# haliphinx/TCE-RVOS

Hardware: AMD Instinct MI355X
Metric: clips/s (T=5, 360×640, Swin-T) at 1/2/4/8 MI355X; mask IoU vs ref (higher is better)
Workload: dtype f32 (3xf16-split MFMA, f32 accumulate); 1 GPU; swin_t_p4w7 T=5 360x640 + 32-token text, B=1 clip per forward, flags --with_box_refine --binary --f_token 8 --qtrans (BASELINE config 2); clips_in_flight_per_gpu=1, clips_per_forward=1, same_clip_in_group=False, ranks_per_gpu=1, parallelism=clip-sharded x1

## Files before the change

include/tce_rvos.h:

```cpp
#ifndef TCE_RVOS_H
#define TCE_RVOS_H
#include <stdint.h>

#ifdef __cplusplus
extern "C" {
#endif

typedef void* tceStream;

int tce_abi_version(void);
const char* tce_last_error(void);

typedef struct {
  const float* A;
  const float* A2;
  const float* W;
  const float* bias;
  const float* res;
  float* C;
  int32_t M, N, K;
  int32_t lda, lda2, ldw, ldc, ldres;
  int32_t act, res_mode;
  int32_t batch;
  int64_t sA, sA2, sW, sBias, sC, sRes;
// ... 114 lines not shown
int tce_embed_ln_f32(const int64_t* ids, const int64_t* pos_ids, const float* word, const float* pos, const float* type0,
                     const float* gamma, const float* beta, float* out, int32_t L, int32_t C, float eps, int32_t pad_id,
                     tceStream stream);
int tce_embed_ln_seqs_f32(const int64_t* ids, const float* word, const float* pos, const float* type0, const float* gamma,
                          const float* beta, float* out, int32_t nseq, int32_t seq_len, int32_t C, float eps, int32_t pad_id,
                          tceStream stream);
int tce_mha_small64_f32(const float* qkv, float* out, int32_t L, int32_t nheads, float scale, tceStream stream);
int tce_tanh_f32(const float* x, float* out, int64_t n, tceStream stream);

int32_t tce_thin_linear_splits(int32_t M, int32_t N, int32_t K);
int tce_thin_partials_f32(const float* x, int64_t ldx, int32_t xsplits, const float* bias_x, int32_t act_x, const float* W,
                          int64_t ldw, float* ws, int32_t M, int32_t N, int32_t K, tceStream stream);
int tce_splitk_reduce_f32(const float* ws, int32_t splits, int32_t M, int32_t N, const float* bias, int32_t act, const float* res,
                          int32_t ldres, int32_t res_mode, float* C, int32_t ldc, const float* gamma, const float* beta, float eps,
                          tceStream stream);
int tce_mha_small64_splits_f32(const float* qkv_planes, int32_t splits, const float* bias, float* out, int32_t L, int32_t nheads,
                               float scale, tceStream stream);
int tce_mha_small64_seqs_f32(const float* qkv_planes, int32_t splits, const float* bias, float* out, int32_t nseq, int32_t L,
                             int32_t nheads, float scale, tceStream stream);
int tce_mha_small64_lens_f32(const float* qkv_planes, int32_t splits, const float* bias, float* out, int32_t nseq, int32_t L,
                             int32_t nheads, float scale, const int32_t* lens, tceStream stream);
int tce_caption_lens_f32(const int64_t* ids, int32_t nseq, int32_t Lmax, int32_t pad_id, int32_t D, int32_t* lens, uint8_t* kmask,
                         float* pos, tceStream stream);

int64_t tce_ffn_packed_bytes(int32_t C, int32_t Hd);
int tce_ffn_pack_f32(const float* W1, const float* b1, const float* W2, void* packed, int32_t C, int32_t Hd,
                     tceStream stream);
int tce_ffn_pack_batched_f32(const float* W1, const float* b1, const float* W2, void* packed, int32_t C, int32_t Hd,
                             int32_t batch, tceStream stream);
int tce_ffn_fused_f32(const float* x, int64_t ldx, const void* packed, const float* b2, const float* g_in,
                      const float* be_in, float eps_in, const float* g_out, const float* be_out, float eps_out,
                      float* out, int64_t ldo, int32_t M, int32_t C, int32_t Hd, int32_t act, tceStream stream);
int64_t tce_ffn_split_ws_floats(int32_t M, int32_t C, int32_t Hd, int32_t act);
int32_t tce_ffn_split_counters(int32_t M, int32_t C, int32_t Hd, int32_t act);
int tce_ffn_fused_split_f32(const float* x, int64_t ldx, const void* packed, const float* b2, const float* g_in, const float* be_in,
                            float eps_in, const float* g_out, const float* be_out, float eps_out, float* out, int64_t ldo, int32_t M,
                            int32_t C, int32_t Hd, int32_t act, float* ws, int64_t ws_floats, int32_t* counters, int32_t n_counters,
                            tceStream stream);

typedef struct {
  const float* x;
  const float* a2;
  const void* packed;
  const float* bias;
  const float* res;
  float* out;
  const float *g_in, *be_in, *g_out, *be_out;
  int64_t ldx, lda2, ldres, ldo;
  int64_t sX, sA2, sRes, sOut;
  int32_t M, N, K, batch, a2_rows, act, res_mode;
  float eps_in, eps_out;
} tceRowLinArgs;
int64_t tce_rowlin_packed_bytes(int32_t N, int32_t K);
int tce_rowlin_pack_f32(const float* W, int64_t ldw, void* packed, int32_t N, int32_t K, tceStream stream);
int tce_rowlin_f32(const tceRowLinArgs* args, tceStream stream);

int64_t tce_conv3x3_packed_bytes(int32_t Cin, int32_t N);
int tce_conv3x3_pack_f32(const float* w, void* packed, int32_t Cin, int32_t N, tceStream stream);
int tce_conv3x3_f32(const float* x, int64_t ldx, const void* packed, const float* bias, float* out, int64_t ldo, int32_t T,
                    int32_t H, int32_t W, int32_t Cin, int32_t N, tceStream stream);
int64_t tce_conv3x3_split_ws_floats(int32_t M, int32_t Cin, int32_t N);
int32_t tce_conv3x3_split_pieces(int32_t M, int32_t Cin, int32_t N);
int32_t tce_conv3x3_split_kstep(int32_t pieces, int32_t s);
int tce_conv3x3_split_f32(const float* x, int64_t ldx, const void* packed, const float* bias, float* out, int64_t ldo, int32_t T,
                          int32_t H, int32_t W, int32_t Cin, int32_t N, float* ws, int64_t ws_floats, tceStream stream);

// ... 77 lines not shown
```

tce-rvos_amd/_lib.py:

```python
import ctypes as C
import os

HERE = os.path.dirname(os.path.abspath(__file__))
LIB_PATH = os.environ.get("TCE_LIB") or os.path.join(HERE, "lib", "libtce_rvos.so")

c_f = C.c_void_p
i32, i64, f32 = C.c_int32, C.c_int64, C.c_float


class GemmArgs(C.Structure):
    _fields_ = [("A", c_f), ("A2", c_f), ("W", c_f), ("bias", c_f), ("res", c_f), ("C", c_f),
                ("M", i32), ("N", i32), ("K", i32),
                ("lda", i32), ("lda2", i32), ("ldw", i32), ("ldc", i32), ("ldres", i32),
                ("act", i32), ("res_mode", i32), ("batch", i32),
                ("sA", i64), ("sA2", i64), ("sW", i64), ("sBias", i64), ("sC", i64), ("sRes", i64),
                ("conv", i32), ("T", i32), ("H", i32), ("Wd", i32), ("Cin", i32), ("Ho", i32), ("Wo", i32),
                ("kh", i32), ("kw", i32), ("stride", i32), ("pad", i32)]


class RowLinArgs(C.Structure):
    _fields_ = [("x", c_f), ("a2", c_f), ("packed", c_f), ("bias", c_f), ("res", c_f), ("out", c_f),
                ("g_in", c_f), ("be_in", c_f), ("g_out", c_f), ("be_out", c_f),
                ("ldx", i64), ("lda2", i64), ("ldres", i64), ("ldo", i64),
                ("sX", i64), ("sA2", i64), ("sRes", i64), ("sOut", i64),
# ... 64 lines not shown
    "tce_ms_deform_attn_forward_f32": (i32, [c_f, c_f, c_f, c_f, c_f, c_f, i32, i32, i32, i32, i32, i32, i32, c_f]),
    "tce_ms_deform_attn_backward_f32": (i32, [c_f, c_f, c_f, c_f, c_f, c_f, c_f, c_f, c_f, i32, i32, i32, i32, i32, i32, i32, c_f]),
    "tce_msda_fused_f32": (i32, [c_f, c_f, c_f, c_f, C.POINTER(i32), i32, i32, i32, i32, i32, i32, i32, i32, c_f]),
    "tce_msda_fused_valid_f32": (i32, [c_f, c_f, c_f, c_f, C.POINTER(i32), C.POINTER(i32), i32, i32, i32, i32, i32, i32, i32,
                                       i32, c_f]),
    "tce_msda_fewq_raw_f32": (i32, [c_f, c_f, c_f, c_f, c_f, c_f, C.POINTER(i32), C.POINTER(i32), i32, i32, i32, i32, i32, i32, i32,
                                    i32, c_f]),
    "tce_contrastive_f32": (i32, [c_f, c_f, c_f, c_f, i32, i32, i32, i32, c_f]),
    "tce_pos_sine2d_f32": (i32, [c_f, c_f, i32, i32, i32, i32, c_f]),
    "tce_pos_sine2d_valid_f32": (i32, [c_f, c_f, i32, i32, i32, i32, i32, i32, c_f]),
    "tce_resize_nearest_f32": (i32, [c_f, c_f, c_f, i32, i32, i32, i32, i32, i32, c_f]),
    "tce_resize_bilinear_f32": (i32, [c_f, c_f, c_f, i32, i32, i32, i32, i32, i32, c_f]),
    "tce_resize_bilinear_ln_f32": (i32, [c_f, c_f, c_f, c_f, f32, c_f, i32, i32, i32, i32, i32, i32, c_f]),
    "tce_add_f32": (i32, [c_f, c_f, c_f, i64, i64, c_f]),
    "tce_tile_f32": (i32, [c_f, c_f, i64, i64, c_f]),
    "tce_sigmoid_f32": (i32, [c_f, c_f, i64, c_f]),
    "tce_copy_segments": (i32, [C.POINTER(CopySeg), i32, c_f]),
    "tce_box_refine_f32": (i32, [c_f, c_f, c_f, i32, i32, c_f]),
    "tce_mask_pack_f32": (i32, [c_f, c_f, c_f, i32, i32, i32, i32, c_f]),
    "tce_mask_tail_f32": (i32, [c_f, c_f, c_f, i32, c_f, i32, i32, i32, i32, i32, f32, f32, i32, c_f]),
    "tce_select_masks_u8": (i32, [c_f, c_f, c_f, c_f, i32, i32, i32, i32, i32, i32, i32, f32, c_f]),
    "tce_embed_ln_f32": (i32, [c_f, c_f, c_f, c_f, c_f, c_f, c_f, c_f, i32, i32, f32, i32, c_f]),
    "tce_mha_small64_f32": (i32, [c_f, c_f, i32, i32, f32, c_f]),
    "tce_mha_small64_seqs_f32": (i32, [c_f, i32, c_f, c_f, i32, i32, i32, f32, c_f]),
    "tce_embed_ln_seqs_f32": (i32, [c_f, c_f, c_f, c_f, c_f, c_f, c_f, i32, i32, i32, f32, i32, c_f]),
    "tce_mha_small64_lens_f32": (i32, [c_f, i32, c_f, c_f, i32, i32, i32, f32, c_f, c_f]),
    "tce_caption_lens_f32": (i32, [c_f, i32, i32, i32, i32, c_f, c_f, c_f, c_f]),
    "tce_tanh_f32": (i32, [c_f, c_f, i64, c_f]),
    "tce_ffn_packed_bytes": (i64, [i32, i32]),
    "tce_ffn_pack_f32": (i32, [c_f, c_f, c_f, c_f, i32, i32, c_f]),
    "tce_ffn_fused_f32": (i32, [c_f, i64, c_f, c_f, c_f, c_f, f32, c_f, c_f, f32, c_f, i64, i32, i32, i32, i32, c_f]),
    "tce_ffn_split_ws_floats": (i64, [i32, i32, i32, i32]),
    "tce_ffn_split_counters": (i32, [i32, i32, i32, i32]),
    "tce_ffn_fused_split_f32": (i32, [c_f, i64, c_f, c_f, c_f, c_f, f32, c_f, c_f, f32, c_f, i64, i32, i32, i32, i32, c_f, i64, c_f, i32, c_f]),
    "tce_xattn_prepare_f32": (i32, [c_f, c_f, c_f, c_f, c_f, c_f, c_f, i32, i32, i32, c_f]),
    "tce_ffn_pack_batched_f32": (i32, [c_f, c_f, c_f, c_f, i32, i32, i32, c_f]),
    "tce_xattn_fused_f32": (i32, [C.POINTER(XattnArgs), c_f]),
    "tce_xattn_ffn_fused_f32": (i32, [C.POINTER(XattnArgs), C.POINTER(XattnFfnArgs), c_f]),
    "tce_ffn_pack_chain_f32": (i32, [c_f, c_f, c_f, c_f, i32, i32, c_f]),
    "tce_xattn_pack_f32": (i32, [c_f, c_f, c_f, c_f, c_f, i32, i32, i32, c_f]),
    "tce_xattn_prepare_lens_f32": (i32, [c_f, c_f, c_f, c_f, c_f, c_f, c_f, i32, i32, i32, c_f, c_f]),
    "tce_xattn_pack_lens_f32": (i32, [c_f, c_f, c_f, c_f, c_f, i32, i32, i32, c_f, c_f]),
    "tce_rowlin_packed_bytes": (i64, [i32, i32]),
    "tce_rowlin_pack_f32": (i32, [c_f, i64, c_f, i32, i32, c_f]),
    "tce_rowlin_f32": (i32, [C.POINTER(RowLinArgs), c_f]),
    "tce_conv3x3_packed_bytes": (i64, [i32, i32]),
    "tce_conv3x3_pack_f32": (i32, [c_f, c_f, i32, i32, c_f]),
    "tce_conv3x3_f32": (i32, [c_f, i64, c_f, c_f, c_f, i64, i32, i32, i32, i32, i32, c_f]),
    "tce_conv3x3_split_ws_floats": (i64, [i32, i32, i32]),
    "tce_conv3x3_split_pieces": (i32, [i32, i32, i32]),
    "tce_conv3x3_split_kstep": (i32, [i32, i32]),
    "tce_conv3x3_split_f32": (i32, [c_f, i64, c_f, c_f, c_f, i64, i32, i32, i32, i32, i32, c_f, i64, c_f]),
    "tce_fewrow_linear_f32": (i32, [C.POINTER(FewRowArgs), c_f]),
    "tce_thin_linear_splits": (i32, [i32, i32, i32]),
    "tce_thin_partials_f32": (i32, [c_f, i64, i32, c_f, i32, c_f, i64, c_f, i32, i32, i32, c_f]),
    "tce_splitk_reduce_f32": (i32, [c_f, i32, i32, i32, c_f, i32, c_f, i32, i32, c_f, i32, c_f, c_f, f32, c_f]),
    "tce_mha_small64_splits_f32": (i32, [c_f, i32, c_f, c_f, i32, i32, f32, c_f]),
    "tce_swin_attn_packed_bytes": (i64, [i32]),
    "tce_swin_attn_pack_f32": (i32, [c_f, c_f, c_f, i32, c_f]),
    "tce_swin_attn_fused_f32": (i32, [c_f, i64, c_f, c_f, c_f, c_f, c_f, c_f, f32, c_f, i64, i32, i32, i32, i32, i32, c_f]),
    "tce_graph_begin": (i32, [c_f]),
    "tce_graph_end": (i32, [c_f, C.POINTER(C.c_void_p)]),
    "tce_graph_launch": (i32, [C.c_void_p, c_f]),
    "tce_graph_destroy": (i32, [C.c_void_p]),
    "tce_graph_group": (i32, [C.POINTER(C.c_void_p), i32, C.POINTER(C.c_void_p)]),
}
# ... 56 lines not shown
```

tce-rvos_amd/csrc/chain.hip:

```cpp
#include "common.h"
#include "gemm_epilogue.h"
#include "frag.h"
#include "../../include/tce_rvos.h"
#include "../../include/tce_rvos_debug.h"

namespace {

#ifndef FFN_ABL
#define FFN_ABL 0
#endif
static __device__ long long* g_ffn_stamps = nullptr;


template <int K, bool HAS_A2 = true>
__device__ __forceinline__ void load_x_frags(const float* __restrict__ x, const long long ldx,
                                             const float* __restrict__ a2, const long long lda2, const int a2_rows,
                                             const int m0, const int M, float* __restrict__ wt, const int lane,
                                             const float* __restrict__ g_in, const float* __restrict__ be_in,
                                             const float eps, h16x8 (&xh)[K / 16], h16x8 (&xl)[K / 16],
                                             const int single = 0) {
  constexpr int NP = K / 32;
  const int cr = lane >> 3, cp = (lane & 7) * 4;
  const int r = lane & 31, hf = lane >> 5;
  f32x4 v[NP][4];
// ... 199 lines not shown
      const f32x4 gv = *reinterpret_cast<const f32x4*>(gamma + 32 * t + 8 * g + 4 * hf);
      const f32x4 bv = *reinterpret_cast<const f32x4*>(beta + 32 * t + 8 * g + 4 * hf);
#pragma unroll
      for (int c = 0; c < 4; ++c) acc[t][4 * g + c] = (acc[t][4 * g + c] - mean) * rstd * gv[c] + bv[c];
    }
}

struct FfnArgs {
  const float* x;
  const unsigned char* wpk;
  const float* b2;
  const float *g_in, *be_in, *g_out, *be_out;
  float* out;
  long long ldx, ldo;
  const float *a2, *res;
  long long lda2, ldres, sX, sRes, sOut, sW;
  int a2_rows, res_mode;
  int M, NI;
  float eps_in, eps_out;
  int* range_flag;
  int single;
  int wdiv;
  const unsigned char* wpk2;
  const float *b22, *g_out2, *be_out2;
  float* mid;
  long long ldmid, sMid;
  int NI2;
  float eps_out2;
  float* ws;
  int* cnt;
  int sp_p, sp_k0, sp_k1, nblk;
};

template <int C, int WAVES, int ACT, bool SINGLE, int ACT2 = 0, bool SPLIT = false>
__global__ void __launch_bounds__(64 * WAVES, (WAVES == 4 && C <= 128) ? 2 : WAVES / 4) ffn_fused_kernel(const FfnArgs p) {
  static_assert(!(SPLIT && ACT2 != 0), "a chain is not split");
  constexpr int KS = C / 16, NT = C / 32;
  constexpr bool HALF = WAVES == 4 && C <= 128;
  constexpr int PWAVES = HALF ? 8 : WAVES;
  constexpr int P = (1 + 2 * KS + 4 * NT + PWAVES - 1) / PWAVES * PWAVES;
  constexpr int SLOTS = P / WAVES;
  static_assert(!(HALF && (SPLIT || ACT2 != 0)), "the half form is the plain kernel");
  constexpr int STAGE = P * PIECE;
  constexpr int STEPS = KS + 2 * NT;
  static_assert(SLOTS <= STEPS, "more DMA slots than loop steps");
  static_assert(2 * STAGE + (HALF ? 0 : WAVES * WT_BYTES) <= (HALF ? 80 : 160) * 1024, "ring + staging tiles do not fit the LDS");
  static_assert(!HALF || WAVES * WT_BYTES <= STAGE, "the half form's staging tiles alias one ring stage");
  __shared__ __attribute__((aligned(16))) unsigned char smem[2 * STAGE + (HALF ? 0 : WAVES * WT_BYTES) + (SPLIT ? 16 : 0)];

  const int tid = threadIdx.x, lane = tid & 63;
  const int wave = __builtin_amdgcn_readfirstlane(tid >> 6);
  const int hf = lane >> 5;

  if (p.NI < 0) reinterpret_cast<u32x4*>(smem)[tid] = u32x4{0u, 0u, 0u, 0u};

  long long* const stamps = (g_ffn_stamps && blockIdx.x < 1024 && blockIdx.y == 0 && tid == 0) ? g_ffn_stamps + blockIdx.x * 8 : nullptr;
  if (stamps) {
    stamps[0] = (long long)__builtin_amdgcn_s_memtime();
    stamps[4] = (long long)__builtin_amdgcn_s_memrealtime();
  }
  const unsigned char* wp = p.wpk + (long long)(blockIdx.y / p.wdiv) * p.sW + (long long)wave * PIECE;
  const unsigned char* const wp0 = wp;
  const unsigned voff = lane * 16;
  const unsigned wbase = wave * PIECE;
  auto dma = [&](int stage, int q) {
    const unsigned char* src = wp;
    if constexpr (ACT2 != 0 || SPLIT) {
      const unsigned long long u = (unsigned long long)wp;
      const unsigned lo = __builtin_amdgcn_readfirstlane((unsigned)u), hi = __builtin_amdgcn_readfirstlane((unsigned)(u >> 32));
      src = (const unsigned char*)(((unsigned long long)hi << 32) | lo);
      glds16(src, voff, (unsigned)__builtin_amdgcn_readfirstlane((int)(wbase + (unsigned)(stage * STAGE + q * WAVES * PIECE))));
      wp += WAVES * PIECE;
      return;
    }
    glds16(src, voff, wbase + (unsigned)(stage * STAGE + q * WAVES * PIECE));
    wp += WAVES * PIECE;
  };
  const float* const xb = p.x + blockIdx.y * p.sX;
  const float* const resb = p.res ? p.res + blockIdx.y * p.sRes : xb;
  const long long ldres = p.res ? p.ldres : p.ldx;
  float* const outb = p.out + blockIdx.y * p.sOut;
  float* const wt = reinterpret_cast<float*>(smem + (HALF ? STAGE : 2 * STAGE) + wave * WT_BYTES);
  tce_amax_t amax = 0;
  constexpr int single = SINGLE;
  constexpr int NPC = SPLIT ? 2 : 1;
  for (int pc = 0; pc < NPC; ++pc) {
  int blk = blockIdx.x, nit = p.NI;
  if constexpr (SPLIT) {
    const int q = p.sp_p + 1, g = blockIdx.x / q, i = blockIdx.x - g * q;
    int c0 = 0;
    if (pc == 0) {
      if (i == p.sp_p) continue;
      blk = g * p.sp_p + i;
      nit = (i == 0 ? p.sp_k0 : p.sp_k1) + 1;
    } else {
      if (i == 0) continue;
      blk = g * p.sp_p + i - 1;
      c0 = i == 1 ? p.sp_k0 : p.sp_k1;
      nit = p.NI - c0;
    }
    if (blk >= p.nblk) continue;
    wp = wp0 + (long long)c0 * (P * PIECE);
  }
#pragma unroll
  for (int q = 0; q < SLOTS; ++q) dma(0, q);

  const int m0 = blk * (32 * WAVES) + wave * 32;
  h16x8 xh[KS], xl[KS];
  load_x_frags<C, (ACT >= 3)>(xb, p.ldx, p.a2, p.lda2, p.a2_rows, m0, p.M, wt, lane, p.g_in, p.be_in, p.eps_in, xh, xl, SINGLE);

  f32x16 oacc[NT];
#pragma unroll
  for (int t = 0; t < NT; ++t)
#pragma unroll
    for (int i = 0; i < 16; ++i) oacc[t][i] = 0.f;
  h16x8 hh0, hl0, hh1, hl1;
#pragma unroll
  for (int j = 0; j < 8; ++j) hh0[j] = hl0[j] = hh1[j] = hl1[j] = (_Float16)0.f;

  asm volatile("s_waitcnt vmcnt(0)" ::: "memory");
// ... 552 lines not shown
inline FfnSplitPlan ffn_split_plan(int M, int C, int Hd, int batch) {
  FfnSplitPlan best;
  const int B = tce_cdiv(M, 32 * ffn_waves(C)), NC = Hd / 32, CUS = tce_cu_count();
  if (C != 256 || NC < 24 || batch < 1) return best;
  const int OVP = 3, OVF = 4;
  auto rounds = [&](long long wgs) { return (double)((wgs + CUS - 1) / CUS); };
  double best_cost = 0.75 * rounds((long long)B * batch) * (NC + 1 + OVP + OVF);
  for (int p = 1; p <= 2; ++p) {
    const int wd = p == 1 ? 0 : (p * NC - 2 * (1 + OVP)) / (p + 1), ws_ = p == 1 ? (NC + 1) / 2 : wd + 1 + OVP;
    int k[2] = {ws_, 0};
    bool ok = ws_ >= 1 && ws_ <= NC - 1;
    for (int i = 1; i < p && ok; ++i) {
      k[i] = wd - (NC - k[i - 1]);
      ok = k[i] >= 1 && k[i] <= NC - 1;
    }
    if (!ok) continue;
    const int busiest = ws_ > NC - k[p - 1] ? ws_ : NC - k[p - 1];
    const double cost = rounds((long long)tce_cdiv(B, p) * (p + 1) * batch) * (busiest + 1 + OVP + OVF);
    if (cost < best_cost) {
      best_cost = cost;
      best.p = p;
      for (int i = 0; i < 2; ++i) best.k[i] = k[i];
    }
  }
  if (best.p) {
    best.nblk = B;
    best.ws_floats = (long long)batch * B * 2 * (32 * ffn_waves(C)) * C;
  }
  return best;
}

static int g_ffn_half = 0;

template <int C, int WAVES>
void ffn_launch(const FfnArgs& a, int act, hipStream_t s, int batch = 1) {
  if constexpr (C == 256) {
    if (a.sp_p > 0 && act == 1) {
      const dim3 grid(tce_cdiv(a.nblk, a.sp_p) * (a.sp_p + 1), batch), block(64 * WAVES);
      if (a.single) hipLaunchKernelGGL((ffn_fused_kernel<C, WAVES, 1, true, 0, true>), grid, block, 0, s, a);
      else hipLaunchKernelGGL((ffn_fused_kernel<C, WAVES, 1, false, 0, true>), grid, block, 0, s, a);
      return;
    }
  }
  if constexpr (C <= 128 && WAVES == 8) {
    const long long b8 = (long long)tce_cdiv(a.M, 256) * batch, b4 = (long long)tce_cdiv(a.M, 128) * batch, cus = tce_cu_count();
    const double c8 = (double)((b8 + cus - 1) / cus);
    const long long rem = b4 % (2 * cus);
    const double c4 = (double)(b4 / (2 * cus)) + (rem == 0 ? 0.0 : rem <= cus ? 0.5 : 1.0);
    if (act == 2 && g_ffn_half >= 0 && (g_ffn_half > 0 || c4 <= c8)) {
      const dim3 grid(tce_cdiv(a.M, 128), batch), block(256);
      if (a.single) hipLaunchKernelGGL((ffn_fused_kernel<C, 4, 2, true>), grid, block, 0, s, a);
      else hipLaunchKernelGGL((ffn_fused_kernel<C, 4, 2, false>), grid, block, 0, s, a);
      return;
    }
  }
  const dim3 grid(tce_cdiv(a.M, 32 * WAVES), batch), block(64 * WAVES);
  if (a.single) {
    if (act == 1) hipLaunchKernelGGL((ffn_fused_kernel<C, WAVES, 1, true>), grid, block, 0, s, a);
    else if (act == 2) hipLaunchKernelGGL((ffn_fused_kernel<C, WAVES, 2, true>), grid, block, 0, s, a);
  } else {
    if (act == 1) hipLaunchKernelGGL((ffn_fused_kernel<C, WAVES, 1, false>), grid, block, 0, s, a);
    else if (act == 2) hipLaunchKernelGGL((ffn_fused_kernel<C, WAVES, 2, false>), grid, block, 0, s, a);
  }
}

__global__ void __launch_bounds__(256) xattn_prepare_kernel(const float* __restrict__ k, const float* __restrict__ v,
                                                            const float* __restrict__ wqT, const float* __restrict__ wo,
                                                            float* __restrict__ W1, float* __restrict__ b1,
                                                            float* __restrict__ W2, const int L, const int G,
                                                            const int* __restrict__ lens) {
  constexpr int C = 256, HD = 32;
  const int Hd = 8 * G;
  const int Lb = lens ? min(lens[blockIdx.y], L) : L;
  k += (long long)blockIdx.y * L * C;
  v += (long long)blockIdx.y * L * C;
  W1 += (long long)blockIdx.y * Hd * C;
  b1 += (long long)blockIdx.y * Hd;
  W2 += (long long)blockIdx.y * C * Hd;
  const int idx = blockIdx.x * 256 + threadIdx.x;
  if (idx < Hd * C) {
    const int r = idx / C, i = idx - r * C, h = r / G, j = r - h * G;
    float a = 0.f;
    if (j < Lb) {
      const f32x4* kp = reinterpret_cast<const f32x4*>(k + j * C + h * HD);
      const f32x4* wp = reinterpret_cast<const f32x4*>(wqT + (long long)i * C + h * HD);
// ... 513 lines not shown
  hipLaunchKernelGGL(ffn_pack_kernel, dim3(tce_cdiv(units, 256)), dim3(256), 0, (hipStream_t)stream, W1, b1, W2,
                     (unsigned char*)packed, C, Hd, ffn_pieces(C), units, tce_gemm_single_pass(), 1);
  TCE_CHECK_LAUNCH("tce_ffn_pack_chain_f32");
  return TCE_OK;
}

extern "C" int tce_ffn_fused_f32(const float* x, int64_t ldx, const void* packed, const float* b2, const float* g_in,
                                 const float* be_in, float eps_in, const float* g_out, const float* be_out,
                                 float eps_out, float* out, int64_t ldo, int32_t M, int32_t C, int32_t Hd, int32_t act,
                                 tceStream stream) {
  TCE_CHECK_ARG(ffn_shape_ok(C, Hd), "tce_ffn_fused_f32: unsupported shape C=%d hidden=%d", C, Hd);
  TCE_CHECK_ARG(M > 0 && x && packed && b2 && out, "tce_ffn_fused_f32: null pointer or M <= 0");
  TCE_CHECK_ARG(act == 1 || act == 2, "tce_ffn_fused_f32: act must be 1 (ReLU) or 2 (GELU)");
  TCE_CHECK_ARG(ldx >= C && ldo >= C && ldx % 4 == 0 && ldo % 4 == 0, "tce_ffn_fused_f32: bad row pitch");
  TCE_CHECK_ARG(tce_aligned16(x) && tce_aligned16(out) && tce_aligned16(packed) && tce_aligned16(b2),
                "tce_ffn_fused_f32: x/out/packed/b2 must be 16-byte aligned");
  TCE_CHECK_ARG((!g_in || (be_in && tce_aligned16(g_in) && tce_aligned16(be_in))) &&
                    (!g_out || (be_out && tce_aligned16(g_out) && tce_aligned16(be_out))),
                "tce_ffn_fused_f32: LayerNorm gamma/beta must come in pairs, 16-byte aligned");
  FfnArgs a = {};
  a.x = x; a.wpk = (const unsigned char*)packed; a.b2 = b2; a.res_mode = 1;
  a.g_in = g_in; a.be_in = be_in; a.g_out = g_out; a.be_out = be_out;
  a.out = out; a.ldx = ldx; a.ldo = ldo; a.M = M; a.NI = Hd / 32 + 1; a.eps_in = eps_in; a.eps_out = eps_out; a.range_flag = tce_range_flag(); a.single = tce_gemm_single_pass();
  a.wdiv = 1;
  hipStream_t s = (hipStream_t)stream;
  if (C == 256) ffn_launch<256, 4>(a, act, s);
  else if (C == 192) ffn_launch<192, 4>(a, act, s);
  else if (C == 128) ffn_launch<128, 8>(a, act, s);
  else ffn_launch<96, 8>(a, act, s);
  TCE_CHECK_LAUNCH("tce_ffn_fused_f32");
  return TCE_OK;
}

extern "C" int tce_debug_ffn_set_half(int32_t mode) {
  TCE_CHECK_ARG(mode >= -1 && mode <= 1, "tce_debug_ffn_set_half: -1 (never), 0 (automatic) or 1 (always)");
  g_ffn_half = mode;
  return TCE_OK;
}

extern "C" int64_t tce_ffn_split_ws_floats(int32_t M, int32_t C, int32_t Hd, int32_t act) {
  if (M <= 0 || !ffn_shape_ok(C, Hd) || act != 1) return 0;
  return ffn_split_plan(M, C, Hd, 1).ws_floats;
}

extern "C" int32_t tce_ffn_split_counters(int32_t M, int32_t C, int32_t Hd, int32_t act) {
  if (M <= 0 || !ffn_shape_ok(C, Hd) || act != 1) return 0;
  return ffn_split_plan(M, C, Hd, 1).nblk;
}

extern "C" int tce_ffn_fused_split_f32(const float* x, int64_t ldx, const void* packed, const float* b2, const float* g_in,
                                       const float* be_in, float eps_in, const float* g_out, const float* be_out, float eps_out,
                                       float* out, int64_t ldo, int32_t M, int32_t C, int32_t Hd, int32_t act, float* ws,
                                       int64_t ws_floats, int32_t* counters, int32_t n_counters, tceStream stream) {
  TCE_CHECK_ARG(ffn_shape_ok(C, Hd), "tce_ffn_fused_split_f32: unsupported shape C=%d hidden=%d", C, Hd);
  TCE_CHECK_ARG(M > 0 && x && packed && b2 && out, "tce_ffn_fused_split_f32: null pointer or M <= 0");
  TCE_CHECK_ARG(act == 1, "tce_ffn_fused_split_f32: act must be 1 (ReLU)");
  TCE_CHECK_ARG(ldx >= C && ldo >= C && ldx % 4 == 0 && ldo % 4 == 0, "tce_ffn_fused_split_f32: bad row pitch");
  TCE_CHECK_ARG(tce_aligned16(x) && tce_aligned16(out) && tce_aligned16(packed) && tce_aligned16(b2),
                "tce_ffn_fused_split_f32: x/out/packed/b2 must be 16-byte aligned");
  TCE_CHECK_ARG((!g_in || (be_in && tce_aligned16(g_in) && tce_aligned16(be_in))) &&
                    (!g_out || (be_out && tce_aligned16(g_out) && tce_aligned16(be_out))),
                "tce_ffn_fused_split_f32: LayerNorm gamma/beta must come in pairs, 16-byte aligned");
  const FfnSplitPlan plan = ffn_split_plan(M, C, Hd, 1);
  TCE_CHECK_ARG(plan.p > 0, "tce_ffn_fused_split_f32: no split is planned for M=%d C=%d hidden=%d (tce_ffn_split_ws_floats is 0): "
                "call tce_ffn_fused_f32", M, C, Hd);
  TCE_CHECK_ARG(ws && tce_aligned16(ws) && ws_floats >= plan.ws_floats && counters && n_counters >= plan.nblk,
// ... 94 lines not shown
static int xattn_launch(const tceXattnArgs* args, const tceXattnFfnArgs* ffn, tceStream stream) {
  TCE_CHECK_ARG(args != nullptr, "tce_xattn_fused_f32: null args");
  const tceXattnArgs& q = *args;
  TCE_CHECK_ARG(q.M > 0 && q.x && q.packed && q.bo && q.out, "tce_xattn_fused_f32: null pointer or M <= 0");
  TCE_CHECK_ARG(q.res_mode == 1 || q.res_mode == 2, "tce_xattn_fused_f32: res_mode must be 1 (add) or 2 (multiply)");
  TCE_CHECK_ARG(q.group == 32 || q.group == 8, "tce_xattn_fused_f32: group (key slots per head) must be 32 or 8");
  TCE_CHECK_ARG(q.ldx >= 256 && q.ldo >= 256 && q.ldx % 4 == 0 && q.ldo % 4 == 0 && (!q.res || (q.ldres >= 256 && q.ldres % 4 == 0)) &&
                    (!q.a2 || (q.lda2 >= 256 && q.lda2 % 4 == 0)) && q.sX % 4 == 0 && q.sRes % 4 == 0 && q.sOut % 4 == 0,
                "tce_xattn_fused_f32: bad row pitch / batch stride");
  TCE_CHECK_ARG(tce_aligned16(q.x) && tce_aligned16(q.out) && tce_aligned16(q.packed) && tce_aligned16(q.bo) &&
                    (!q.a2 || tce_aligned16(q.a2)) && (!q.res || tce_aligned16(q.res)),
                "tce_xattn_fused_f32: pointers must be 16-byte aligned");
  TCE_CHECK_ARG(!q.g_out || (q.be_out && tce_aligned16(q.g_out) && tce_aligned16(q.be_out)),
                "tce_xattn_fused_f32: LayerNorm gamma/beta must come in pairs, 16-byte aligned");
  FfnArgs a = {};
  a.x = q.x; a.wpk = (const unsigned char*)q.packed; a.b2 = q.bo; a.g_out = q.g_out; a.be_out = q.be_out; a.out = q.out;
  a.ldx = q.ldx; a.ldo = q.ldo; a.a2 = q.a2; a.lda2 = q.lda2; a.a2_rows = q.a2_rows; a.res = q.res; a.ldres = q.ldres;
  a.res_mode = q.res_mode; a.sX = q.sX; a.sRes = q.sRes; a.sOut = q.sOut; a.sW = q.sW;
  a.M = q.M; a.NI = (8 * q.group) / 32 + 1; a.eps_out = q.eps_out; a.range_flag = tce_range_flag(); a.single = tce_gemm_single_pass();
  a.wdiv = q.w_div > 0 ? q.w_div : 1;
  const int batch = q.batch > 0 ? q.batch : 1;
  const dim3 grid(tce_cdiv(a.M, 128), batch), block(256);
  if (ffn) {
    a.wpk2 = (const unsigned char*)ffn->packed; a.b22 = ffn->b2; a.g_out2 = ffn->g_out; a.be_out2 = ffn->be_out; a.eps_out2 = ffn->eps_out;
    a.mid = ffn->mid; a.ldmid = ffn->ldmid; a.sMid = ffn->sMid; a.NI2 = ffn->hidden / 32 + 1;
    if (a.single) {
      if (q.group == 32) hipLaunchKernelGGL((ffn_fused_kernel<256, 4, 3, true, 1>), grid, block, 0, (hipStream_t)stream, a);
      else hipLaunchKernelGGL((ffn_fused_kernel<256, 4, 4, true, 1>), grid, block, 0, (hipStream_t)stream, a);
    } else {
      if (q.group == 32) hipLaunchKernelGGL((ffn_fused_kernel<256, 4, 3, false, 1>), grid, block, 0, (hipStream_t)stream, a);
      else hipLaunchKernelGGL((ffn_fused_kernel<256, 4, 4, false, 1>), grid, block, 0, (hipStream_t)stream, a);
    }
    TCE_CHECK_LAUNCH("tce_xattn_ffn_fused_f32");
    return TCE_OK;
  }
  if (a.single) {
    if (q.group == 32) hipLaunchKernelGGL((ffn_fused_kernel<256, 4, 3, true>), grid, block, 0, (hipStream_t)stream, a);
    else hipLaunchKernelGGL((ffn_fused_kernel<256, 4, 4, true>), grid, block, 0, (hipStream_t)stream, a);
  } else {
    if (q.group == 32) hipLaunchKernelGGL((ffn_fused_kernel<256, 4, 3, false>), grid, block, 0, (hipStream_t)stream, a);
    else hipLaunchKernelGGL((ffn_fused_kernel<256, 4, 4, false>), grid, block, 0, (hipStream_t)stream, a);
  }
  TCE_CHECK_LAUNCH("tce_xattn_fused_f32");
  return TCE_OK;
}

#endif

#if TCE_CHAIN_PART != 1
int tce_chain_rowlin_set_stamps(long long* dev_buf) {
  return hipMemcpyToSymbol(HIP_SYMBOL(g_ffn_stamps), &dev_buf, sizeof(dev_buf)) == hipSuccess ? 0 : -1;
}

extern "C" int64_t tce_rowlin_packed_bytes(int32_t N, int32_t K) { return rowlin_shape_ok(N, K) ? rowlin_units(N, K) * 16 : -1; }

extern "C" int tce_rowlin_pack_f32(const float* W, int64_t ldw, void* packed, int32_t N, int32_t K, tceStream stream) {
  TCE_CHECK_ARG(rowlin_shape_ok(N, K), "tce_rowlin_pack_f32: unsupported shape N=%d K=%d (K in 96/128/192/256/384/512, N %% 32 == 0)", N, K);
  TCE_CHECK_ARG(W && packed && tce_aligned16(packed) && ldw >= K, "tce_rowlin_pack_f32: null / misaligned pointer or ldw < K");
  const long long units = rowlin_units(N, K);
  hipLaunchKernelGGL(rowlin_pack_kernel, dim3(tce_cdiv(units, 256)), dim3(256), 0, (hipStream_t)stream, W,
                     (unsigned char*)packed, N, K, (long long)ldw, units, tce_gemm_single_pass());
  TCE_CHECK_LAUNCH("tce_rowlin_pack_f32");
  return TCE_OK;
}

extern "C" int tce_rowlin_f32(const tceRowLinArgs* args, tceStream stream) {
// ... 187 lines not shown
```

tce-rvos_amd/hazard.py:

```python
import contextlib
import traceback

import numpy as np
import torch

from . import _lib

F = 4


def strided(ptr, run_bytes, *dims):
    if not ptr or run_bytes <= 0 or any(c <= 0 for c, _ in dims):
        return np.zeros((0, 2), dtype=np.int64)
    starts = np.array([int(ptr)], dtype=np.int64)
    for count, stride in dims:
        if count == 1 or stride == 0:
            continue
        starts = (starts[:, None] + (np.arange(int(count), dtype=np.int64) * int(stride))[None, :]).reshape(-1)
    iv = np.stack([starts, starts + int(run_bytes)], 1)
    return merge(iv)


def dense(ptr, nbytes):
    return strided(ptr, int(nbytes))
# ... 373 lines not shown
    "tce_mha_small64_splits_f32": lambda a: ([dense(_p(a[0]), a[1] * a[4] * 3 * a[5] * 64 * F), dense(_p(a[2]), 3 * a[5] * 64 * F)],
                                             [dense(_p(a[3]), a[4] * a[5] * 64 * F)]),
    "tce_mha_small64_seqs_f32": lambda a: ([dense(_p(a[0]), a[1] * a[4] * a[5] * 3 * a[6] * 64 * F), dense(_p(a[2]), 3 * a[6] * 64 * F)],
                                           [dense(_p(a[3]), a[4] * a[5] * a[6] * 64 * F)]),
    "tce_mha_small64_lens_f32": lambda a: ([dense(_p(a[0]), a[1] * a[4] * a[5] * 3 * a[6] * 64 * F), dense(_p(a[2]), 3 * a[6] * 64 * F),
                                            dense(_p(a[8]), a[4] * 4)],
                                           [dense(_p(a[3]), a[4] * a[5] * a[6] * 64 * F)]),
    "tce_caption_lens_f32": lambda a: ([dense(_p(a[0]), a[1] * a[2] * 8)],
                                       [dense(_p(a[5]), a[1] * 4), dense(_p(a[6]), a[1] * a[2]), dense(_p(a[7]), a[1] * a[2] * a[4] * F)]),
    "tce_embed_ln_seqs_f32": lambda a: _embed(a[0], None, a[1], a[2], a[3], a[4], a[5], a[6], a[7] * a[8], a[9], a[11], a[8]),
    "tce_swin_attn_pack_f32": lambda a: ([dense(_p(a[0]), 3 * a[3] * a[3] * F), dense(_p(a[1]), a[3] * a[3] * F)],
                                         [dense(_p(a[2]), _lib.lib_raw().tce_swin_attn_packed_bytes(a[3]))]),
    "tce_swin_attn_fused_f32": lambda a: (
        [strided(_p(a[0]), a[14] * F, (a[11] * a[12] * a[13], a[1] * F)), dense(_p(a[2]), _lib.lib_raw().tce_swin_attn_packed_bytes(a[14])),
         dense(_p(a[3]), 3 * a[14] * F), dense(_p(a[4]), a[14] * F), dense(_p(a[5]), 169 * (a[14] // 32) * F),
         dense(_p(a[6]), a[14] * F), dense(_p(a[7]), a[14] * F)],
        [strided(_p(a[9]), a[14] * F, (a[11] * a[12] * a[13], a[10] * F))]),
}


def _label_objects(a):
    objs, n, labels, best, T, Q, K, h, w, H0, W0 = a[:11]
    rd = []
    for i in range(n):
        rd += [dense(_p(objs[i].logits), T * Q * K * F), dense(_p(objs[i].masks), T * Q * h * w * F)]
    return rd, [dense(_p(labels), T * H0 * W0), dense(_p(best), n * 4)]


VIDEO_MODELS = {
    "tce_label_objects_u8": _label_objects,
}
NOT_LAUNCHES = {"tce_abi_version", "tce_last_error", "tce_gemm_select_tile", "tce_gemm_select_tile_ex", "tce_set_gemm_mode", "tce_set_gemm_mode_thread",
                "tce_get_gemm_mode", "tce_set_range_flag", "tce_groupnorm_nsplit", "tce_mha_ws_bytes", "tce_ffn_packed_bytes", "tce_ffn_split_ws_floats", "tce_ffn_split_counters",
                "tce_rowlin_packed_bytes", "tce_conv3x3_packed_bytes", "tce_conv3x3_split_ws_floats",
                "tce_conv3x3_split_pieces", "tce_conv3x3_split_kstep", "tce_swin_attn_packed_bytes", "tce_thin_linear_splits", "tce_graph_begin", "tce_graph_end", "tce_graph_launch",
                "tce_graph_destroy", "tce_graph_group"} | set(_lib.DEBUG_SIGNATURES)


class Launch:
    __slots__ = ("idx", "name", "stream", "tick", "clock", "reads", "writes", "site")

    def __repr__(self):
        return f"#{self.idx} {self.name} on stream {self.stream:#x} at {self.site}"


class Recorder:

    def __init__(self):
        self.launches = []
        self.clock = {}
        self.events = {}
        self.edges = 0
        self.host_syncs = 0

    def _clk(self, s):
        c = self.clock.get(int(s))
        if c is None:
            c = self.clock[int(s)] = dict(getattr(self, "_future", {}))
        return c

    def launch(self, name, stream, reads, writes, site):
        s = int(stream or 0)
        c = self._clk(s)
        c[s] = c.get(s, 0) + 1
        L = Launch()
        L.idx, L.name, L.stream, L.tick, L.clock = len(self.launches), name, s, c[s], dict(c)
# ... 155 lines not shown
```

tce-rvos_amd/ops.py:

```python
import ctypes as C

import os
import threading

import torch

from ._lib import GemmArgs, check, lib

ACT_NONE, ACT_RELU, ACT_GELU, ACT_RELU_AFTER_RES = 0, 1, 2, 3
RES_NONE, RES_ADD, RES_MUL = 0, 1, 2


class Arena:

    ALIGN = 256
    FLAGS = 1 << 14

    def __init__(self, device, nbytes):
        self.device = torch.device(device)
        self.buf = torch.empty(int(nbytes), dtype=torch.uint8, device=self.device)
        self.off = 0
        self.peak = 0
        self.flags = torch.zeros(self.FLAGS, dtype=torch.int32, device=self.device)
        self.flag_off = 0
# ... 54 lines not shown
    e1.record()
    b = max(1, g.batch)
    GEMM_PROFILE.append((lib().tce_gemm_select_tile_ex(g.M, g.N, g.K, b, g.conv), bool(g.conv), 2.0 * g.M * g.N * g.K * b, e0, e1))


def set_gemm_mode(mode):
    check(lib().tce_set_gemm_mode({"f32": 0, "f16x3": 1, "f16": 2}[mode]), "tce_set_gemm_mode")


def get_gemm_mode():
    return {0: "f32", 1: "f16x3", 2: "f16"}[lib().tce_get_gemm_mode()]


_ARITH_TL = threading.local()


class arith:

    def __init__(self, mode):
        self.mode, self.prev = mode, None

    def __enter__(self):
        if self.mode is not None:
            self.prev = getattr(_ARITH_TL, "mode", None)
            _ARITH_TL.mode = self.mode
            check(lib().tce_set_gemm_mode_thread({"f32": 0, "f16x3": 1, "f16": 2}[self.mode]), "tce_set_gemm_mode_thread")
        return self

    def __exit__(self, *exc):
        if self.mode is not None:
            _ARITH_TL.mode = self.prev
            check(lib().tce_set_gemm_mode_thread(-1 if self.prev is None else {"f32": 0, "f16x3": 1, "f16": 2}[self.prev]),
                  "tce_set_gemm_mode_thread")
        return False


def _stream():
    return torch.cuda.current_stream().cuda_stream


FP16_RANGE_LIMIT = 60000.0
_RANGE = {}


class RangeError(RuntimeError):
    pass


def range_flag(device=None):
    dev = torch.device("cuda", torch.cuda.current_device()) if device is None else torch.device(device)
    if dev.index is None:
        dev = torch.device("cuda", torch.cuda.current_device())
    st = _RANGE.get(dev)
    if st is None:
        st = {"flag": torch.zeros(1, dtype=torch.int32, device=dev), "host": torch.zeros(1, dtype=torch.int32).pin_memory(),
              "event": None}
        _RANGE[dev] = st
        check(lib().tce_set_range_flag(st["flag"].data_ptr()), "tce_set_range_flag")
    return st


def range_snapshot_async(device=None):
    st = range_flag(device)
    st["host"].copy_(st["flag"], non_blocking=True)
    st["event"] = torch.cuda.Event()
    st["event"].record()
# ... 1077 lines not shown
```

tce-rvos_amd/pipeline.py:

```python
import os

import torch

from . import ops
from .ops import ACT_GELU, ACT_RELU, ACT_RELU_AFTER_RES, RES_ADD, RES_MUL, gemm_ex

D = 256
NH = 8
FFN_FUSED_MIN_ROWS = int(__import__("os").environ.get("TCE_FFN_FUSED_MIN_ROWS", 16000))
SWIN_FUSED_MIN_TOKENS = int(os.environ.get("TCE_SWIN_FUSED_MIN_TOKENS", 2000))


def _proj_res_ln(x, wt, bias, resid, M, norm_w, norm_b):
    pk = ops.rowlin_lookup(wt, D, D) if M >= FFN_FUSED_MIN_ROWS else None
    if pk is not None:
        ops.rowlin(x, pk, resid, M, D, D, D, D, bias=bias, res=resid, ldres=D, res_mode=RES_ADD, ln_out=(norm_w, norm_b))
        return
    gemm_ex(x, wt, resid, M, D, D, D, D, D, bias=bias, res=resid, ldres=D, res_mode=RES_ADD)
    ops.layernorm(resid, norm_w, norm_b, 1e-5, out=resid)


def _lin(A, x, M, K, w, b, N, **kw):
    out = A(M, N)
    gemm_ex(x, w, out, M, N, K, K, K, N, bias=b, **kw)
    return out


ABLATE = set(filter(None, os.environ.get("TCE_ABLATE", "").split(",")))
TAPS = os.environ.get("TCE_TAPS") == "1"
FEWROW_OK = os.environ.get("TCE_FEWROW", "1") != "0"
FEWROW_SITES = os.environ["TCE_FEWROW_SITES"].split(",") if "TCE_FEWROW_SITES" in os.environ else None
TEXT_LATE = os.environ.get("TCE_TEXT_LATE", "1") != "0"
TEXT_EARLY_EDGE = os.environ.get("TCE_TEXT_EARLY_EDGE", "0") != "0"
EARLY_PROJ = os.environ.get("TCE_EARLY_PROJ", "1") != "0"
TOKFORK = os.environ.get("TCE_TOKFORK", "1") != "0"
ENCFORK = os.environ.get("TCE_ENCFORK", "1") != "0"
DEFER_OUT_NORM = os.environ.get("TCE_DEFER_OUT_NORM", "1") != "0"
LAT1_AT = os.environ.get("TCE_LAT1_AT")
SWIN3_FC2_SPLITK = int(os.environ.get("TCE_SWIN3_FC2_SPLITK", 2))
FTF_LN_FUSE = os.environ.get("TCE_FTF_LN_FUSE", "0") != "0"
if ABLATE or TAPS:
    import warnings
    warnings.warn(f"tce_rvos_amd: DIAGNOSTIC launch program (TCE_ABLATE={sorted(ABLATE)}, TCE_TAPS={int(TAPS)}): "
                  + ("stages are skipped, every result of this process is GARBAGE" if ABLATE else "intermediates are copied out"),
                  RuntimeWarning, stacklevel=2)


_TAP_FN = None

STAGE_EVENTS = None


def _stage(name):
    if STAGE_EVENTS is not None:
        e = torch.cuda.Event(enable_timing=True)
        e.record()
        STAGE_EVENTS.append((name, e))


class _Fork:

    def __init__(self, side_stream, after=None):
        self.side = side_stream
        self.after = after
        self.ctx = None

    def __enter__(self):
        if self.side is not None:
            if self.after is not None:
                self.side.wait_event(self.after)
            else:
# ... 179 lines not shown
            s = _lin(A, feat, T * hw, chs[1 + l], w[f"input_proj.{l}.0.weight"], w[f"input_proj.{l}.0.bias"], D)
        else:
            h5, w5 = sizes[3]
            k5 = 9 * chs[3]
            sk = next((c for c in (8, 6, 4, 3, 2) if k5 % (c * 32) == 0), 1) if T * h * ww <= 2048 else 1
            s, ho, wo = ops.conv2d_cl(feat, w["input_proj.3.0.weight:cl"], T, h5, w5, chs[3], 3, 3, 2, 1,
                                      bias=w["input_proj.3.0.bias"], alloc=A, splitk=sk,
                                      ws=A(sk * T * h * ww * D) if sk > 1 else None)
            assert (ho, wo) == (h, ww)
        s = ops.groupnorm_cl(s, w[f"input_proj.{l}.1.weight"], w[f"input_proj.{l}.1.bias"], T, hw, D, 32, alloc=A)
        if fpk is not None and Tc * hw >= ops.XATTN_MIN_ROWS:
            ops.xattn_fused(s, fpk, w["fusion_module.multihead_attn.out_proj.bias"], hw, src[starts[l]:], res_mode=RES_MUL,
                            batch=T, sX=hw * D, sRes=hw * D, sOut=S * D, per_batch_weights=G > 1, w_div=Tc)
        else:
            q = _lin(A, s, T * hw, D, w["fusion_module.multihead_attn.q.w"], w["fusion_module.multihead_attn.q.b"], D)
            att = A(T * hw, D)
            ops.mha_core(q, fk, fv, G, NH, Tc * hw, L, D, D, D, Tc * hw * D, L * D, L * D, att, D, Tc * hw * D, kmask=fkm)
            gemm_ex(att, w["fusion_module.multihead_attn.out_proj.weight"], src[starts[l]:], hw, D, D, D, D, D,
                    bias=w["fusion_module.multihead_attn.out_proj.bias"], res=s, ldres=D, res_mode=RES_MUL, batch=T,
                    sA=hw * D, sC=S * D, sRes=hw * D)

    ar2, stream2 = fork2 if fork2 is not None else (None, None)
    lat1 = None
    if early:
        for arx, _ in fork3:
            arx.reset()

    def pick(feat, i):
        if select is None:
            return feat
        hw_i = sizes[i][0] * sizes[i][1]
        return feat[select * hw_i:(select + 1) * hw_i]

    pending_norm0 = []

    def on_stage(i, feat, finish=None):
        if i == 0 and text_late:
            text_stage()
        if i == 0 and finish is not None:
            pending_norm0.append(finish)
        feat = pick(feat, i)
        if early:
            if i in (1, 2):
                    arx, stx = fork3[i - 1]
                    fk_ = _Fork(stx)
                    with fk_:
                        if finish is not None:
                            finish()
                        text_fork.join()
                        input_level(i - 1, feat, arx.alloc)
                    lvl_forks.append(fk_)
    if DEFER_OUT_NORM:
        on_stage.defers = lambda i: select is None and ((i == 0 and ar2 is not None and stream2 is not None) or (i in (1, 2) and early))
    if cfg.is_resnet:
        with model.arith("backbone.merge"):
            feats = _resnet_backbone(model, frames, ar, sizes, rep=G if shared else 1)
    else:
        feats = _swin_backbone(model, frames, ar, sizes, on_stage, 1 if shared else G, rep=G if shared else 1)
    feats = [pick(f, i) for i, f in enumerate(feats)]

    _stage("backbone")
    text_fork.join()
    _stage("text join")

    def start_lat1():
        ar2.reset()
        lat1_fork = _Fork(stream2)
        with lat1_fork:
            while pending_norm0:
                pending_norm0.pop()()
            return (lat1_fork, _lateral(model, sc, feats, None, vl_sites, T, L, ffn, ln_, 1, ar2, G))
    lat1_when = LAT1_AT or (f"enc{cfg.enc_layers - 2}" if cfg.enc_layers >= 2 else "backbone")
    if ar2 is not None and stream2 is not None and lat1_when == "backbone":
        lat1 = start_lat1()
    if src is None:
        src = A(T * S, D)
    m_levels = ar.mark()
    if early:
        todo = ((2, side_stream), (3, None))
    else:
        todo = ((1, side_stream), (2, side_stream), (3, side_stream), (0, None))
    for l, lvl_stream in todo:
        fk_ = _Fork(lvl_stream)
        lvl_forks.append(fk_)
        with fk_:
            input_level(l, feats[min(1 + l, 3)], A)
    for fk_ in lvl_forks:
        fk_.join()
    ar.release(m_levels)

    _stage("input_proj + fusion")
    lvl_pos, enc_ref = sc["lvl_pos"], sc["enc_ref"]
    Fk = cfg.f_token
    if Fk > 0:
        token = ops.tile(w["transformer.encoder.memory_bus"], T, out=A(T * Fk, D))
        tpos = w["transformer.encoder.memory_pos"]
        ftf_fuse_ln = FTF_LN_FUSE and D == 256 and all(few(T * Fk, site) for site in ("msda", "ftf2", "ftf3"))
        token_alt = A(T * Fk, D) if ftf_fuse_ln else None
    tok_stream = side_stream if TOKFORK else None

    def msda(pre, query, q_rows, q_per_frame, q_pos, q_pos_shared, value_src, ref, ref_dim, ref_per_frame, resid,
             ar=ar, norm=None, small_fork=None, group="encoder.msda", defer_norm=False):
        with model.arith(group):
            _msda(pre, query, q_rows, q_per_frame, q_pos, q_pos_shared, value_src, ref, ref_dim, ref_per_frame, resid, ar, norm,
                  small_fork, defer_norm)

# ... 667 lines not shown
```

Measured before the change: 172.0 clips/s.

## Cap lateral FFN workgroups with persistent kernel and start lateral branch at backbone

Adds a persistent variant of the fused FFN kernel that loops over row blocks, so the grid can be capped at a set number of workgroups. The lateral-1 branch on the side stream runs with a default cap of 64 WGs when the problem is large enough. With the cap on, that branch launches right after the backbone instead of near the end of the encoder. The goal is to overlap lateral work with the encoder without starving its CUs. In exchange, the capped lateral branch may run slower and could land on the critical path.

```diff
diff --git a/include/tce_rvos.h b/include/tce_rvos.h
--- a/include/tce_rvos.h
+++ b/include/tce_rvos.h
@@ -170,6 +170,8 @@
                       const float* be_in, float eps_in, const float* g_out, const float* be_out, float eps_out,
                       float* out, int64_t ldo, int32_t M, int32_t C, int32_t Hd, int32_t act, tceStream stream);
 int64_t tce_ffn_split_ws_floats(int32_t M, int32_t C, int32_t Hd, int32_t act);
+int tce_ffn_set_wg_cap(int32_t cap);
+int32_t tce_ffn_capped_grid(int32_t cap, int32_t batch, int32_t blocks, int32_t* persistent);
 int32_t tce_ffn_split_counters(int32_t M, int32_t C, int32_t Hd, int32_t act);
 int tce_ffn_fused_split_f32(const float* x, int64_t ldx, const void* packed, const float* b2, const float* g_in, const float* be_in,
                             float eps_in, const float* g_out, const float* be_out, float eps_out, float* out, int64_t ldo, int32_t M,
diff --git a/tce-rvos_amd/_lib.py b/tce-rvos_amd/_lib.py
--- a/tce-rvos_amd/_lib.py
+++ b/tce-rvos_amd/_lib.py
@@ -120,6 +120,8 @@
     "tce_ffn_fused_f32": (i32, [c_f, i64, c_f, c_f, c_f, c_f, f32, c_f, c_f, f32, c_f, i64, i32, i32, i32, i32, c_f]),
     "tce_ffn_split_ws_floats": (i64, [i32, i32, i32, i32]),
     "tce_ffn_split_counters": (i32, [i32, i32, i32, i32]),
+    "tce_ffn_set_wg_cap": (i32, [i32]),
+    "tce_ffn_capped_grid": (i32, [i32, i32, i32, C.POINTER(i32)]),
     "tce_ffn_fused_split_f32": (i32, [c_f, i64, c_f, c_f, c_f, c_f, f32, c_f, c_f, f32, c_f, i64, i32, i32, i32, i32, c_f, i64, c_f, i32, c_f]),
     "tce_xattn_prepare_f32": (i32, [c_f, c_f, c_f, c_f, c_f, c_f, c_f, i32, i32, i32, c_f]),
     "tce_ffn_pack_batched_f32": (i32, [c_f, c_f, c_f, c_f, i32, i32, i32, c_f]),
diff --git a/tce-rvos_amd/csrc/chain.hip b/tce-rvos_amd/csrc/chain.hip
--- a/tce-rvos_amd/csrc/chain.hip
+++ b/tce-rvos_amd/csrc/chain.hip
@@ -255,9 +255,10 @@
   int sp_p, sp_k0, sp_k1, nblk;
 };
 
-template <int C, int WAVES, int ACT, bool SINGLE, int ACT2 = 0, bool SPLIT = false>
+template <int C, int WAVES, int ACT, bool SINGLE, int ACT2 = 0, bool SPLIT = false, bool PERSIST = false>
 __global__ void __launch_bounds__(64 * WAVES, (WAVES == 4 && C <= 128) ? 2 : WAVES / 4) ffn_fused_kernel(const FfnArgs p) {
   static_assert(!(SPLIT && ACT2 != 0), "a chain is not split");
+  static_assert(!PERSIST || (!SPLIT && ACT2 == 0 && !(WAVES == 4 && C <= 128)), "the persistent form is the plain kernel, staging tiles of its own");
   constexpr int KS = C / 16, NT = C / 32;
   constexpr bool HALF = WAVES == 4 && C <= 128;
   constexpr int PWAVES = HALF ? 8 : WAVES;
@@ -307,8 +308,13 @@
   tce_amax_t amax = 0;
   constexpr int single = SINGLE;
   constexpr int NPC = SPLIT ? 2 : 1;
-  for (int pc = 0; pc < NPC; ++pc) {
+  const int npass = PERSIST ? ((p.M + 32 * WAVES - 1) / (32 * WAVES) - (int)blockIdx.x + (int)gridDim.x - 1) / (int)gridDim.x : NPC;
+  for (int pc = 0; pc < (PERSIST ? npass : NPC); ++pc) {
   int blk = blockIdx.x, nit = p.NI;
+  if constexpr (PERSIST) {
+    blk += pc * (int)gridDim.x;
+    wp = wp0;
+  }
   if constexpr (SPLIT) {
     const int q = p.sp_p + 1, g = blockIdx.x / q, i = blockIdx.x - g * q;
     int c0 = 0;
@@ -927,6 +933,17 @@
 
 static int g_ffn_half = 0;
 
+struct FfnGridPlan {
+  int grid_x, persist;
+};
+inline FfnGridPlan ffn_grid_plan(int cap, int batch, int blocks) {
+  if (cap <= 0 || batch < 1 || (long long)blocks * batch <= cap) return {blocks, 0};
+  const int gx = cap / batch > 1 ? cap / batch : 1;
+  if (gx >= blocks) return {blocks, 0};
+  return {gx, 1};
+}
+[[maybe_unused]] static thread_local int t_ffn_wg_cap = 0;
+
 template <int C, int WAVES>
 void ffn_launch(const FfnArgs& a, int act, hipStream_t s, int batch = 1) {
   if constexpr (C == 256) {
@@ -946,6 +963,15 @@
       const dim3 grid(tce_cdiv(a.M, 128), batch), block(256);
       if (a.single) hipLaunchKernelGGL((ffn_fused_kernel<C, 4, 2, true>), grid, block, 0, s, a);
       else hipLaunchKernelGGL((ffn_fused_kernel<C, 4, 2, false>), grid, block, 0, s, a);
+      return;
+    }
+  }
+  if constexpr (C == 256) {
+    const FfnGridPlan gp = ffn_grid_plan(t_ffn_wg_cap, batch, tce_cdiv(a.M, 32 * WAVES));
+    if (gp.persist && act == 1) {
+      const dim3 grid(gp.grid_x, batch), block(64 * WAVES);
+      if (a.single) hipLaunchKernelGGL((ffn_fused_kernel<C, WAVES, 1, true, 0, false, true>), grid, block, 0, s, a);
+      else hipLaunchKernelGGL((ffn_fused_kernel<C, WAVES, 1, false, 0, false, true>), grid, block, 0, s, a);
       return;
     }
   }
@@ -1525,6 +1551,18 @@
   return TCE_OK;
 }
 
+extern "C" int tce_ffn_set_wg_cap(int32_t cap) {
+  TCE_CHECK_ARG(cap >= 0, "tce_ffn_set_wg_cap: cap must be >= 0 (0 = none)");
+  t_ffn_wg_cap = cap;
+  return TCE_OK;
+}
+
+extern "C" int32_t tce_ffn_capped_grid(int32_t cap, int32_t batch, int32_t blocks, int32_t* persistent) {
+  const FfnGridPlan gp = ffn_grid_plan(cap, batch, blocks);
+  if (persistent) *persistent = gp.persist;
+  return gp.grid_x;
+}
+
 extern "C" int tce_debug_ffn_set_half(int32_t mode) {
   TCE_CHECK_ARG(mode >= -1 && mode <= 1, "tce_debug_ffn_set_half: -1 (never), 0 (automatic) or 1 (always)");
   g_ffn_half = mode;
@@ -1685,6 +1723,19 @@
       else hipLaunchKernelGGL((ffn_fused_kernel<256, 4, 4, false, 1>), grid, block, 0, (hipStream_t)stream, a);
     }
     TCE_CHECK_LAUNCH("tce_xattn_ffn_fused_f32");
+    return TCE_OK;
+  }
+  const FfnGridPlan gp = ffn_grid_plan(t_ffn_wg_cap, batch, tce_cdiv(a.M, 128));
+  if (gp.persist) {
+    const dim3 pgrid(gp.grid_x, batch);
+    if (a.single) {
+      if (q.group == 32) hipLaunchKernelGGL((ffn_fused_kernel<256, 4, 3, true, 0, false, true>), pgrid, block, 0, (hipStream_t)stream, a);
+      else hipLaunchKernelGGL((ffn_fused_kernel<256, 4, 4, true, 0, false, true>), pgrid, block, 0, (hipStream_t)stream, a);
+    } else {
+      if (q.group == 32) hipLaunchKernelGGL((ffn_fused_kernel<256, 4, 3, false, 0, false, true>), pgrid, block, 0, (hipStream_t)stream, a);
+      else hipLaunchKernelGGL((ffn_fused_kernel<256, 4, 4, false, 0, false, true>), pgrid, block, 0, (hipStream_t)stream, a);
+    }
+    TCE_CHECK_LAUNCH("tce_xattn_fused_f32");
     return TCE_OK;
   }
   if (a.single) {
diff --git a/tce-rvos_amd/hazard.py b/tce-rvos_amd/hazard.py
--- a/tce-rvos_amd/hazard.py
+++ b/tce-rvos_amd/hazard.py
@@ -429,6 +429,7 @@
 }
 NOT_LAUNCHES = {"tce_abi_version", "tce_last_error", "tce_gemm_select_tile", "tce_gemm_select_tile_ex", "tce_set_gemm_mode", "tce_set_gemm_mode_thread",
                 "tce_get_gemm_mode", "tce_set_range_flag", "tce_groupnorm_nsplit", "tce_mha_ws_bytes", "tce_ffn_packed_bytes", "tce_ffn_split_ws_floats", "tce_ffn_split_counters",
+                "tce_ffn_set_wg_cap", "tce_ffn_capped_grid",
                 "tce_rowlin_packed_bytes", "tce_conv3x3_packed_bytes", "tce_conv3x3_split_ws_floats",
                 "tce_conv3x3_split_pieces", "tce_conv3x3_split_kstep", "tce_swin_attn_packed_bytes", "tce_thin_linear_splits", "tce_graph_begin", "tce_graph_end", "tce_graph_launch",
                 "tce_graph_destroy", "tce_graph_group"} | set(_lib.DEBUG_SIGNATURES)
diff --git a/tce-rvos_amd/ops.py b/tce-rvos_amd/ops.py
--- a/tce-rvos_amd/ops.py
+++ b/tce-rvos_amd/ops.py
@@ -110,6 +110,25 @@
             _ARITH_TL.mode = self.prev
             check(lib().tce_set_gemm_mode_thread(-1 if self.prev is None else {"f32": 0, "f16x3": 1, "f16": 2}[self.prev]),
                   "tce_set_gemm_mode_thread")
+        return False
+
+
+class ffn_wg_cap:
+
+    def __init__(self, n):
+        self.n, self.prev = int(n or 0), 0
+
+    def __enter__(self):
+        self.prev = getattr(_ARITH_TL, "wg_cap", 0)
+        if self.n != self.prev:
+            _ARITH_TL.wg_cap = self.n
+            check(lib().tce_ffn_set_wg_cap(self.n), "tce_ffn_set_wg_cap")
+        return self
+
+    def __exit__(self, *exc):
+        if self.n != self.prev:
+            _ARITH_TL.wg_cap = self.prev
+            check(lib().tce_ffn_set_wg_cap(self.prev), "tce_ffn_set_wg_cap")
         return False
 
 
diff --git a/tce-rvos_amd/pipeline.py b/tce-rvos_amd/pipeline.py
--- a/tce-rvos_amd/pipeline.py
+++ b/tce-rvos_amd/pipeline.py
@@ -37,6 +37,9 @@
 ENCFORK = os.environ.get("TCE_ENCFORK", "1") != "0"
 DEFER_OUT_NORM = os.environ.get("TCE_DEFER_OUT_NORM", "1") != "0"
 LAT1_AT = os.environ.get("TCE_LAT1_AT")
+LAT1_CUS = int(os.environ["TCE_LAT1_CUS"]) if os.environ.get("TCE_LAT1_CUS", "") != "" else None
+LAT1_CUS_DEFAULT = 64
+LAT1_CUS_MIN_BLOCKS = 563
 SWIN3_FC2_SPLITK = int(os.environ.get("TCE_SWIN3_FC2_SPLITK", 2))
 FTF_LN_FUSE = os.environ.get("TCE_FTF_LN_FUSE", "0") != "0"
 if ABLATE or TAPS:
@@ -282,14 +285,32 @@
         hw_i = sizes[i][0] * sizes[i][1]
         return feat[select * hw_i:(select + 1) * hw_i]
 
+    lat1_cap = LAT1_CUS
+    if lat1_cap is None:
+        measured = G == 1 and not cfg.is_resnet and not cfg.video and -(-(T * sizes[0][0] * sizes[0][1]) // 128) >= LAT1_CUS_MIN_BLOCKS
+        lat1_cap = LAT1_CUS_DEFAULT if measured else 0
     pending_norm0 = []
 
+    def start_lat1(feat0=None, wait_text=False):
+        ar2.reset()
+        lat1_fork = _Fork(stream2)
+        with lat1_fork:
+            while pending_norm0:
+                pending_norm0.pop()()
+            if wait_text:
+                text_fork.join()
+            with ops.ffn_wg_cap(lat1_cap):
+                return (lat1_fork, _lateral(model, sc, feats if feat0 is None else [feat0], None, vl_sites, T, L, ffn, ln_, 1, ar2, G))
+
     def on_stage(i, feat, finish=None):
+        nonlocal lat1
         if i == 0 and text_late:
             text_stage()
         if i == 0 and finish is not None:
             pending_norm0.append(finish)
         feat = pick(feat, i)
+        if i == 0 and LAT1_AT == "text" and ar2 is not None and stream2 is not None:
+            lat1 = start_lat1(feat, wait_text=True)
         if early:
             if i in (1, 2):
                     arx, stx = fork3[i - 1]
@@ -313,15 +334,8 @@
     text_fork.join()
     _stage("text join")
 
-    def start_lat1():
-        ar2.reset()
-        lat1_fork = _Fork(stream2)
-        with lat1_fork:
-            while pending_norm0:
-                pending_norm0.pop()()
-            return (lat1_fork, _lateral(model, sc, feats, None, vl_sites, T, L, ffn, ln_, 1, ar2, G))
-    lat1_when = LAT1_AT or (f"enc{cfg.enc_layers - 2}" if cfg.enc_layers >= 2 else "backbone")
-    if ar2 is not None and stream2 is not None and lat1_when == "backbone":
+    lat1_when = LAT1_AT or (f"enc{cfg.enc_layers - 2}" if cfg.enc_layers >= 2 and lat1_cap <= 0 else "backbone")
+    if ar2 is not None and stream2 is not None and lat1 is None and lat1_when in ("backbone", "text"):
         lat1 = start_lat1()
     if src is None:
         src = A(T * S, D)
```

Result: faster. 177.0 clips/s (median of 6 runs) (+2.9%).
